# baaivision/Painter

Measured on AMD Instinct MI355X. Metric: images/sec (896x448 pairs) ViT-L fwd+bwd, higher is better.
Workload: dtype bf16; 1 GPU; painter_vit_large_patch16_input896x448 bf16 batch=8/GPU fwd+bwd on 1xMI355X (BASELINE configs[1]); global_batch=8, image=896x448x3 stitched pair, mode=train (DropPath 0.1), parallelism=dp1, rccl_ranks=0, backend=n/a, grad_allreduce=n/a

## Files before the change

include/painter_hip.h:

```cpp
#ifndef PAINTER_HIP_H
#define PAINTER_HIP_H

#include <stdint.h>

#ifdef __cplusplus
extern "C" {
#endif

#ifndef __HIP__
typedef struct ihipStream_t* hipStream_t;
#endif

enum { PA_F32 = 0, PA_BF16 = 1 };
enum {
    PA_EPI_BIAS = 0,
    PA_EPI_BIAS_F32 = 1,
    PA_EPI_BIAS_GELU = 2,
    PA_EPI_BIAS_RESID = 3
};

#define PA_ABI_VERSION 9
int pa_abi_version(void);
int pa_debug_set(int which, int value);
int pa_debug_get(int which);
// ... 5 lines not shown
int pa_linear_fwd_skip(int dtype, int epilogue, const void* x, int64_t ldx, const void* w, const float* bias, void* out, void* out2,
                       int64_t ldo, const float* resid, const float* rowscale, int rows_per_sample, int M, int N, int K,
                       const float* rowskip, int skip_rows_per_sample, hipStream_t stream);
int pa_linear_pixshuf(int dtype, const void* x, int64_t ldx, const void* w , const float* bias,
                      void* out_nhwc, int batch, int Hp, int Wp, int P, int C, int K, hipStream_t stream);
int64_t pa_linear_dgrad_workspace_bytes(int M, int K);
int pa_linear_dgrad(int dtype, const void* dy , int64_t lddy, const void* w ,
                    const void* gelu_aux , void* dx , int64_t lddx, float* dx_colsum,
                    void* workspace, int M, int N, int K, hipStream_t stream);
int pa_linear_dgrad_skip(int dtype, const void* dy, int64_t lddy, const void* w, const void* gelu_aux, void* dx, int64_t lddx, float* dx_colsum,
                         void* workspace, int M, int N, int K, const float* rowskip , int skip_rows_per_sample,
                         hipStream_t stream);
int64_t pa_linear_wgrad_workspace_bytes(int dtype, int M, int N, int K);
int pa_linear_wgrad(int dtype, const void* dy , int64_t lddy, const void* x , int64_t ldx,
                    float* dw , void* workspace, int M, int N, int K, hipStream_t stream);
int64_t pa_colsum_workspace_bytes(int M, int N);
int pa_colsum(int dtype, const void* x , int64_t ld, int M, int N, float* out , void* workspace,
              hipStream_t stream);
int pa_slab_reduce(const float* in, float* out, int64_t n, int nz, int64_t stride, int accumulate, hipStream_t stream);

int pa_layernorm_fwd(int dtype, const float* x, int64_t ldx, const float* gamma, const float* beta, float eps,
                     void* y , int64_t ldy, float* mean, float* rstd,
                     int R, int D, hipStream_t stream);
int64_t pa_layernorm_bwd_workspace_bytes(int R, int D);
int pa_layernorm_bwd(int dtype, const void* dy, int64_t lddy, const float* x, int64_t ldx, const float* mean,
                     const float* rstd, const float* gamma, const float* dres, float* dx, int64_t lddx, void* dxT,
                     int64_t lddxT, const float* rowscale, int rows_per_sample, float* dgamma_dbeta, float* dxT_colsum,
                     void* workspace, int R, int D, hipStream_t stream);
int pa_layernorm_bwd_reduce(const void* workspace, float* dgamma_dbeta, float* dxT_colsum, int with_colsum, int R, int D,
                            hipStream_t stream);
// ... 283 lines not shown
```

painter_amd/_lib.py:

```python
import ctypes
import os
import re

HERE = os.path.dirname(os.path.abspath(__file__))
HEADER = os.path.join(os.path.dirname(HERE), "include", "painter_hip.h")
LIB_PATH = os.environ.get("PAINTER_AMD_LIB") or os.path.join(HERE, "lib", "libpainter_hip.so")

PA_F32, PA_BF16 = 0, 1
EPI_BIAS, EPI_BIAS_F32, EPI_BIAS_GELU, EPI_BIAS_RESID = 0, 1, 2, 3
(KNOB_G256_STAGGER, KNOB_G256_NOSTORE, KNOB_G256_ORDER, KNOB_WGRAD_TARGET, KNOB_G256_SHORT_TILES, KNOB_G256_ILV, KNOB_RELPOS_SPLITS,
 KNOB_ATTN3_FUSE, KNOB_ATTN_LIGHT_LAST, KNOB_CONV_WGRAD_GROUPS, KNOB_LN_BWD_VARIANT, KNOB_G256_PATCH, KNOB_G256_MIXED) = range(13)
KNOB_G256_MIXED_NFULL, KNOB_DROP_SKIP, KNOB_DECODER_ROWS, KNOB_COUNT = 14, 16, 17, 18

_CT = {"int": ctypes.c_int, "int64_t": ctypes.c_int64, "float": ctypes.c_float, "double": ctypes.c_double, "hipStream_t": ctypes.c_void_p}


def parse_header(path=HEADER):
    src = open(path).read()
    src = re.sub(r"/\*.*?\*/", " ", src, flags=re.S)
    src = re.sub(r"//[^\n]*", " ", src)
    protos = {}
    for m in re.finditer(r"\b(int64_t|int)\s+(pa_\w+)\s*\(([^)]*)\)\s*;", src):
        ret, name, args = m.group(1), m.group(2), m.group(3).strip()
        argtypes = []
        if args and args != "void":
            for a in args.split(","):
                a = a.strip()
# ... 47 lines not shown
```

painter_amd/csrc/common.h:

```cpp
#pragma once
#include <hip/hip_runtime.h>
#include <stdint.h>
#include <cstdlib>

typedef __bf16 bf16;
typedef __attribute__((ext_vector_type(8))) __bf16 bf16x8;
typedef __attribute__((ext_vector_type(16))) float f32x16;

#define DEVI __device__ __forceinline__

template <typename T> struct TT;
template <> struct TT<float> {
    static constexpr int EPC = 4;
    static constexpr int BK = 32;
    static constexpr int KSTEPS = 2;
    static constexpr int SPF = 2;
    typedef uint4 Vec4;
};
template <> struct TT<bf16> {
    static constexpr int EPC = 8;
    static constexpr int BK = 64;
    static constexpr int KSTEPS = 4;
    static constexpr int SPF = 1;
    typedef uint2 Vec4;
// ... 69 lines not shown

enum Knob {
    KNOB_G256_STAGGER = 0,
    KNOB_G256_NOSTORE = 1,
    KNOB_G256_ORDER = 2,
    KNOB_WGRAD_TARGET = 3,
    KNOB_G256_SHORT_TILES = 4,
    KNOB_G256_ILV = 5,
    KNOB_RELPOS_SPLITS = 6,
    KNOB_ATTN3_FUSE = 7,
    KNOB_ATTN_LIGHT_LAST = 8,
    KNOB_CONV_WGRAD_GROUPS = 9,
    KNOB_LN_BWD_VARIANT = 10,
    KNOB_G256_PATCH = 11,
    KNOB_G256_MIXED = 12,
    KNOB_FREE_13 = 13,
    KNOB_G256_MIXED_NFULL = 14,
    KNOB_FREE_15 = 15,
    KNOB_DROP_SKIP = 16,
    KNOB_DECODER_ROWS = 17,
    KNOB_COUNT = 18
};
inline int g_knob[KNOB_COUNT] = {};
static inline bool drop_skip_on() {
    static const int env = [] { const char* v = getenv("PAINTER_AMD_DROP_SKIP"); return v ? atoi(v) : 1; }();
    return g_knob[KNOB_DROP_SKIP] == 1 ? false : (g_knob[KNOB_DROP_SKIP] == 2 ? true : env != 0);
}
static inline bool decoder_rows_on() {
    static const int env = [] { const char* v = getenv("PAINTER_AMD_DECODER_ROWS"); return v ? atoi(v) : 1; }();
    return g_knob[KNOB_DECODER_ROWS] == 1 ? false : (g_knob[KNOB_DECODER_ROWS] == 2 ? true : env != 0);
}

inline long long g_attn_counts[6] = {0, 0, 0, 0, 0, 0};
// ... 84 lines not shown
```

painter_amd/csrc/gemm.hip:

```cpp
#include <cstdlib>
#include "gemm_engine.h"
#include "gemm256.h"
#include "../../include/painter_hip.h"

template <typename OutT> struct EpiBias {
    OutT* out; size_t ldo; const float* bias; int M, N;
    DEVI void operator()(const f32x16 (&acc)[2][2], int ib, int jb, int lane, int) const {
        foreach_acc(acc, ib, jb, lane, [&](int i, int j, float v) {
            if (i < M && j < N) out[(size_t)i * ldo + j] = from_f<OutT>(v + (bias ? bias[j] : 0.f));
        });
    }
};
constexpr float G8_OFF = 0.13f, G8_SCALE = 255.f / 1.26f, G8_STEP = 1.26f / 255.f;
DEVI uint32_t g8_code(float g) { return min((uint32_t)fmaf(g, G8_SCALE, G8_OFF * G8_SCALE + 0.5f), 255u); }
DEVI float g8_value(uint32_t q) { return fmaf((float)q, G8_STEP, -G8_OFF); }
template <typename T> struct GeluAux { typedef T type; };
template <> struct GeluAux<bf16> { typedef unsigned char type; };
template <typename T> struct EpiBiasGelu {
    typename GeluAux<T>::type* aux; T* act; size_t ld; const float* bias; int M, N;
    DEVI void operator()(const f32x16 (&acc)[2][2], int ib, int jb, int lane, int) const {
        foreach_acc(acc, ib, jb, lane, [&](int i, int j, float v) {
            if (i < M && j < N) {
                const T p = from_f<T>(v + bias[j]);
                if constexpr (std::is_same<T, bf16>::value) {
// ... 490 lines not shown
extern "C" int pa_linear_dgrad(int dtype, const void* dy, int64_t lddy, const void* w, const void* gelu_aux,
                               void* dx, int64_t lddx, float* dx_colsum, void* workspace, int M, int N, int K, hipStream_t st) {
    return pa_linear_dgrad_skip(dtype, dy, lddy, w, gelu_aux, dx, lddx, dx_colsum, workspace, M, N, K, nullptr, 1, st);
}

static bool wgrad_fast(int dtype, int M, int N, int K) {
    return dtype == PA_BF16 && g256::ok(N, K, M, true, true, N, K) && K % 4 == 0 && N % 256 == 0 && K % 256 == 0;
}
static int wgrad_fast_splits(int M, int N, int K) {
    const int tiles = (N / 256) * (K / 256);
    static const int env_target = [] { const char* v = getenv("PA_WGRAD_WGS"); return v ? atoi(v) : 0; }();
    int target = env_target > 0 ? env_target : (g_knob[KNOB_WGRAD_TARGET] > 0 ? g_knob[KNOB_WGRAD_TARGET] : 256);
    if (target < 16) target = 16;
    int s = (target + 3 * tiles / 4) / tiles;
    if (s < 1) s = 1;
    const int ktiles = M / 64;
    if (s > ktiles / 4) s = ktiles / 4 > 0 ? ktiles / 4 : 1;
    return g256::splits_used(M, s);
}
static int wgrad_splits(int M, int N, int K, int bk) {
    const int tiles = ((N + 127) / 128) * ((K + 127) / 128);
    const int nku = (M + bk - 1) / bk;
    int s = (640 + tiles - 1) / tiles;
    if (s > nku) s = nku;
    if (s > 64) s = 64;
    if (s < 1) s = 1;
    return s;
}
extern "C" int64_t pa_linear_wgrad_workspace_bytes(int dtype, int M, int N, int K) {
    if (wgrad_fast(dtype, M, N, K)) {
        const int s = wgrad_fast_splits(M, N, K);
        return s > 1 ? (int64_t)s * N * K * sizeof(float) : 0;
    }
    const int s = wgrad_splits(M, N, K, dtype == PA_BF16 ? 64 : 32);
    return s > 1 ? (int64_t)s * N * K * sizeof(float) : 0;
}
template <typename T>
static int linear_wgrad_t(const T* dy, int64_t lddy, const T* x, int64_t ldx, float* dw, float* ws, int M, int N, int K,
                          hipStream_t st) {
    if constexpr (std::is_same<T, bf16>::value) {
        if (wgrad_fast(PA_BF16, M, N, K) && g256::ok(N, K, M, true, true, lddy, ldx)) {
            const int s = wgrad_fast_splits(M, N, K);
            if (s == 1) return g256::launch<true, true>(dy, lddy, x, ldx, Epi4Slab{dw, (size_t)K, 0, N, K}, N, K, M, 1, st);
            int e = g256::launch<true, true>(dy, lddy, x, ldx, Epi4Slab{ws, (size_t)K, (size_t)N * K, N, K}, N, K, M, s, st);
            if (e) return e;
            return pa_slab_reduce(ws, dw, (int64_t)N * K, s, (int64_t)N * K, 0, st);
        }
    }
    OpT<T> A{dy, (size_t)lddy, N, 0};
    OpT<T> B{x, (size_t)ldx, K, 0};
    const int s = wgrad_splits(M, N, K, TT<T>::BK);
    if (s == 1) return launch_gemm<T, 2, 2>(A, B, EpiSlab{dw, (size_t)K, 0, N, K}, N, K, M, 1, 1, st);
    int e = launch_gemm<T, 2, 2>(A, B, EpiSlab{ws, (size_t)K, (size_t)N * K, N, K}, N, K, M, s, 1, st);
    if (e) return e;
    return pa_slab_reduce(ws, dw, (int64_t)N * K, s, (int64_t)N * K, 0, st);
}
extern "C" int pa_linear_wgrad(int dtype, const void* dy, int64_t lddy, const void* x, int64_t ldx, float* dw,
                               void* workspace, int M, int N, int K, hipStream_t st) {
    if (N % 4 || K % 4) return (int)hipErrorInvalidValue;
    if (dtype == PA_BF16) return linear_wgrad_t<bf16>((const bf16*)dy, lddy, (const bf16*)x, ldx, dw, (float*)workspace, M, N, K, st);
    return linear_wgrad_t<float>((const float*)dy, lddy, (const float*)x, ldx, dw, (float*)workspace, M, N, K, st);
}

extern "C" int pa_fill_dead_rows(void* x, int64_t pitch_bytes, int64_t row_bytes, const int* rowmap, int M, hipStream_t st);
extern "C" int pa_linear_dgrad_live(const void* dy, int64_t lddy, const void* w, void* dx, int64_t lddx, const int* live, const int* rowmap,
                                    const int* count, int M, int N, int K, hipStream_t st) {
    if (live == nullptr || rowmap == nullptr || count == nullptr || M < 8 || K % 8 || lddx % 8) return (int)hipErrorInvalidValue;
    if (!g256::ok(M, K, N, false, true, lddy, K)) return (int)hipErrorInvalidValue;
    int e = pa_fill_dead_rows(dx, lddx * 2, (int64_t)K * 2, rowmap, M, st);
    if (e) return e;
    return g256::launch_live<false, true>((const bf16*)dy, lddy, (const bf16*)w, K, Epi4Scatter{(bf16*)dx, (size_t)lddx, live, count, M, K}, M, K, N, count, st);
}
extern "C" int pa_linear_wgrad_live(const void* dy, int64_t lddy, const void* x, int64_t ldx, float* dw, const int* count, int M, int N, int K,
                                    hipStream_t st) {
    if (count == nullptr || M < 128 || M % 128) return (int)hipErrorInvalidValue;
    if (!wgrad_fast(PA_BF16, M, N, K) || !g256::ok(N, K, M, true, true, lddy, ldx)) return (int)hipErrorInvalidValue;
// ... 13 lines not shown
```

painter_amd/csrc/gemm256.h:

```cpp
#pragma once
#include "common.h"
#include <cstdlib>
#include <type_traits>

namespace g256 {

constexpr int BM = 256, BN = 256, BK = 64, NT = 512;
constexpr int LDS_BYTES = 131072;
typedef __attribute__((address_space(3))) void lds_void;
typedef __attribute__((address_space(1))) const void gbl_cvoid;

DEVI constexpr int unit_off(bool isB, int sub, int stage) { return (isB ? 65536 : 0) + sub * 32768 + stage * 16384; }

template <int N> DEVI void wait_vm() { asm volatile("s_waitcnt vmcnt(%0)" ::"n"(N) : "memory"); }
DEVI void wait_lgkm0() { asm volatile("s_waitcnt lgkmcnt(0)" ::: "memory"); }

template <bool MM, bool IS_A>
DEVI uint32_t src_off(int tid, int j, int sub, int tile0, int rows, uint32_t ld) {
    const int cidx = j * NT + tid;
    if constexpr (!MM) {
        const int u = cidx >> 3, p = cidx & 7;
        const int kc = p ^ ((u >> 1) & 7);
        int row = IS_A ? ((u >> 6) * 128 + sub * 64 + (u & 63)) : ((u >> 5) * 64 + sub * 32 + (u & 31));
        row = min(tile0 + row, rows - 1);
// ... 51 lines not shown
    template <int KS> DEVI bf16x8 k() const {
        typedef __attribute__((ext_vector_type(2))) uint32_t u2;
        typedef __attribute__((ext_vector_type(4))) uint32_t u4;
        const uint2 l = KS == 0 ? l0 : KS == 1 ? l1 : KS == 2 ? l2 : l3;
        const uint2 h = KS == 0 ? h0 : KS == 1 ? h1 : KS == 2 ? h2 : h3;
        u2 lv = {l.x, l.y}, hv = {h.x, h.y};
        return __builtin_bit_cast(bf16x8, __builtin_shufflevector(lv, hv, 0, 1, 2, 3));
    }
};

template <class Epi> struct epi_colsum { static constexpr bool value = false; };
template <class Epi, class = void> struct epi_hi_off { static constexpr int value = 4; };
template <class Epi> struct epi_hi_off<Epi, std::void_t<decltype(Epi::HI_OFF)>> { static constexpr int value = Epi::HI_OFF; };
constexpr int BM_SHORT = 224;
constexpr int BM_HALF = 128;
template <bool AMM, bool BMM, int ILV, class Epi, bool SHORT = false, bool MIXED = false, bool SKIP = false, bool LIVE = false>
__global__ __launch_bounds__(NT) void gemm256_kernel(const bf16* __restrict__ Ag, uint32_t lda, const bf16* __restrict__ Bg,
                                                      uint32_t ldb, Epi epi, int M, int N, int ktiles, int ktiles_per_split,
                                                      int tiles_n, int stagger, int order, int nfull, int patch,
                                                      const float* __restrict__ rowskip, int rps, const int* __restrict__ live_count) {
    static_assert(!(LIVE && (SHORT || MIXED || SKIP)), "a device-side count goes with uniform 256-row tiles");
    static_assert(!(SHORT && AMM), "the 224-row tile is built for a K-major A operand");
    static_assert(!(SKIP && AMM), "row tiles are skipped only for a K-major A operand");
    static_assert(!(MIXED && (AMM || SHORT)), "half tiles are built for a K-major A operand and 256-row full tiles");
    constexpr int BMR = SHORT ? BM_SHORT : BM;
    extern __shared__ __attribute__((aligned(1024))) unsigned char smem[];
    const int tid = threadIdx.x, lane = tid & 63;
    if (stagger > 0 && blockIdx.x < 256 && blockIdx.y == 0) {
        const int64_t wait = ((int64_t)stagger * (((blockIdx.x >> 3) * 5) & 15)) >> 4;
        const uint64_t t0 = __builtin_amdgcn_s_memtime();
        while ((int64_t)(__builtin_amdgcn_s_memtime() - t0) < wait) __builtin_amdgcn_s_sleep(16);
    }
    const int wv = __builtin_amdgcn_readfirstlane(tid >> 6);
    const int wr = wv >> 2, wc = wv & 3;

    const bool htile = MIXED && (int)blockIdx.x >= nfull * tiles_n;
    int nwg = MIXED ? (htile ? (int)gridDim.x - nfull * tiles_n : nfull * tiles_n) : (int)gridDim.x;
    if constexpr (LIVE) {
        if constexpr (AMM) {
            ktiles = ktiles_per_split = min(ktiles, ((*live_count + 127) >> 7) * 2);
        } else {
            M = min(M, *live_count);
// ... 67 lines not shown
        if (skipped) {
            const int d = bid - nwg;
            int r = d / tiles_n;
            tn = d - r * tiles_n;
            bool found = false;
            skipped_ranges([&](int a, int b) {
                if (!found && r < b - a) { tm = a + r; found = true; }
                if (!found) r -= b - a;
            });
        } else {
            skipped_ranges([&](int a, int b) { if (tm >= a) tm += b - a; });
        }
    }
    const int i0 = htile ? nfull * BMR + tm * BM_HALF : tm * BMR, j0 = tn * BN;
    const bool blk3 = !(SHORT && wr == 1);
    const int kt0 = split * ktiles_per_split;
    const int nt = min(ktiles - kt0, ktiles_per_split);
    const bool empty = LIVE && AMM && nt == 0;
    uint32_t oa[2][2], ob[2][2];
#pragma unroll
    for (int sub = 0; sub < 2; ++sub)
#pragma unroll
        for (int j = 0; j < 2; ++j) {
            oa[sub][j] = src_off<AMM, true>(tid, j, sub, i0, M, lda);
            ob[sub][j] = src_off<BMM, false>(tid, j, sub, j0, N, ldb);
        }
    const size_t a_step = AMM ? (size_t)BK * lda * 2 : (size_t)BK * 2;
    const size_t b_step = BMM ? (size_t)BK * ldb * 2 : (size_t)BK * 2;
    const unsigned char* abase = reinterpret_cast<const unsigned char*>(Ag) + (size_t)kt0 * a_step;
    const unsigned char* bbase = reinterpret_cast<const unsigned char*>(Bg) + (size_t)kt0 * b_step;
    unsigned char* const dma_dst = smem + wv * 1024;

    auto piece_a = [&](int sub, int stage, int kt, int j) {
        const unsigned char* s = sgpr_ptr(abase + (size_t)kt * a_step);
        dma16(s + oa[sub][j], dma_dst + unit_off(false, sub, stage) + j * 8192);
    };
    auto piece_b = [&](int sub, int stage, int kt, int j) {
        const unsigned char* s = sgpr_ptr(bbase + (size_t)kt * b_step);
        dma16(s + ob[sub][j], dma_dst + unit_off(true, sub, stage) + j * 8192);
    };
    auto stage_a = [&](int sub, int stage, int kt) { piece_a(sub, stage, kt, 0); piece_a(sub, stage, kt, 1); };
    auto stage_b = [&](int sub, int stage, int kt) { piece_b(sub, stage, kt, 0); piece_b(sub, stage, kt, 1); };

    uint32_t ra[4], rb[4];
    {
// ... 48 lines not shown
    auto pre = [&](auto&& d0, auto&& d1) {
        if constexpr (ILV < 2) d0();
        if constexpr (ILV < 1) d1();
        wait_vm<8 - ILV>();
    };
    auto bar = [&]() {
        __builtin_amdgcn_sched_barrier(0);
        __builtin_amdgcn_s_barrier();
        __builtin_amdgcn_sched_barrier(0);
    };
    auto lwait = [&]() {
        wait_lgkm0();
        __builtin_amdgcn_sched_barrier(0);
    };

    auto tile_body = [&](auto stage_c, int T) {
        constexpr int S = decltype(stage_c)::value;
        const int t1 = min(T + 1, nt - 1), t2 = min(T + 2, nt - 1);
        fa0.template read<unit_off(false, 0, S)>(ra, 0);
        fa1.template read<unit_off(false, 0, S) + (AMM ? 0 : 4096)>(ra, 1);
        fb0.template read<unit_off(true, 0, S) - 65536>(rb, 0);
        {
            auto d0 = [&] { piece_b(1, S ^ 1, t1, 0); };
            auto d1 = [&] { piece_b(1, S ^ 1, t1, 1); };
            pre(d0, d1);
            bar(); lwait();
            mma_quad(0, 0, fb0, d0, d1);
            bar();
        }
        fb1.template read<unit_off(true, 1, S) - 65536>(rb, 0);
        {
            auto d0 = [&] { piece_a(1, S ^ 1, t1, 0); };
            auto d1 = [&] { piece_a(1, S ^ 1, t1, 1); };
// ... 60 lines not shown
    if constexpr (MIXED) {
        if (htile) {
            ran_half = true;
            if (!skipped) {
                piece_a(0, 0, 0, 0); piece_a(1, 0, 0, 0); stage_b(0, 0, 0); stage_b(1, 0, 0);
                wait_vm<0>();
                bar();
                for (int T = 0; T < nt; T += 2) {
                    half_body(I0{}, T);
                    half_body(I1{}, T + 1);
                }
            }
        }
    }
    if (!ran_half && !skipped && !empty) {
        stage_a(0, 0, 0);
        stage_b(0, 0, 0);
        stage_b(1, 0, 0);
        stage_a(1, 0, 0);
        stage_a(0, 1, 1);
        stage_b(0, 1, 1);
        wait_vm<8>();
        bar();
        if (wr == 1) bar();

        for (int T = 0; T < nt; T += 2) {
            tile_body(I0{}, T);
            tile_body(I1{}, T + 1);
        }
    }
    if (wr == 0 && !ran_half && !skipped && !empty) bar();
    wait_vm<0>();

    bar();
    {
        float* stg = reinterpret_cast<float*>(smem + wv * 8704);
// ... 45 lines not shown
                float v = cs[e];
                v += lane_dpp<0x128>(v);
                v += lane_xor16(v);
                v += lane_xor32(v);
                cs[e] = v;
            }
            if (lane < 8) epi.colsum_out((htile ? nfull + tm : tm) * 2 + wr, jcol, cs);
        }
    }
}

static inline int per_split(int ktiles, int nsplit) {
    int per = (ktiles + nsplit - 1) / nsplit;
    return per + (per & 1);
}
template <bool AMM, bool BMM, int ILV, bool SHORT, class Epi, bool MIXED = false, bool SKIP = false, bool LIVE = false>
static int launch_ilv(const bf16* A, size_t lda, const bf16* B, size_t ldb, Epi epi, int M, int N, int K, int nsplit, hipStream_t st, int nfull = 0,
                      const float* rowskip = nullptr, int rps = 1, const int* live_count = nullptr);
#ifndef G256_ILV_DEFAULT
#define G256_ILV_DEFAULT 2
#endif
static inline bool use_short(int M, int N, int nsplit, bool amm) {
    if (amm || nsplit != 1 || M < BM) return false;
    if (g_knob[KNOB_G256_SHORT_TILES] == 1) return false;
    if (g_knob[KNOB_G256_SHORT_TILES] == 2) return true;
    static const int cost = [] { const char* v = getenv("PA_G256_SHORT_COST"); return v ? atoi(v) : 92; }();
    const int tiles_n = (N + BN - 1) / BN;
    const long t256 = (long)((M + BM - 1) / BM) * tiles_n, t224 = (long)((M + BM_SHORT - 1) / BM_SHORT) * tiles_n;
    const long r256 = (t256 + 255) / 256 * 100, r224 = (t224 + 255) / 256 * cost;
    return r224 < r256;
}
// ... 35 lines not shown
    return launch_ilv<AMM, BMM, G256_ILV_DEFAULT, false>(A, lda, B, ldb, epi, M, N, K, nsplit, st);
#endif
}
template <bool BMM, class Epi>
static int launch_skip(const bf16* A, size_t lda, const bf16* B, size_t ldb, Epi epi, int M, int N, int K, hipStream_t st, const float* rowskip, int rps) {
    if ((M + rps - 1) / rps > 63) return launch<false, BMM>(A, lda, B, ldb, epi, M, N, K, 1, st);
    const TilePlan tp = tile_plan(M, N, 1, false);
    if (tp.mixed) return launch_ilv<false, BMM, G256_ILV_DEFAULT, false, Epi, true, true>(A, lda, B, ldb, epi, M, N, K, 1, st, tp.nfull, rowskip, rps);
    if (tp.is_short) return launch_ilv<false, BMM, G256_ILV_DEFAULT, true, Epi, false, true>(A, lda, B, ldb, epi, M, N, K, 1, st, 0, rowskip, rps);
    return launch_ilv<false, BMM, G256_ILV_DEFAULT, false, Epi, false, true>(A, lda, B, ldb, epi, M, N, K, 1, st, 0, rowskip, rps);
}
template <bool AMM, bool BMM, class Epi>
static int launch_live(const bf16* A, size_t lda, const bf16* B, size_t ldb, Epi epi, int M, int N, int K, const int* live_count, hipStream_t st) {
    return launch_ilv<AMM, BMM, G256_ILV_DEFAULT, false, Epi, false, false, true>(A, lda, B, ldb, epi, M, N, K, 1, st, 0, nullptr, 1, live_count);
}
template <bool AMM, bool BMM, int ILV, bool SHORT, class Epi, bool MIXED, bool SKIP, bool LIVE>
static int launch_ilv(const bf16* A, size_t lda, const bf16* B, size_t ldb, Epi epi, int M, int N, int K, int nsplit, hipStream_t st, int nfull,
                      const float* rowskip, int rps, const int* live_count) {
    auto kern = gemm256_kernel<AMM, BMM, ILV, Epi, SHORT, MIXED, SKIP, LIVE>;
    static bool attr_done = false;
    if (!attr_done) {
        hipError_t e = hipFuncSetAttribute(reinterpret_cast<const void*>(kern), hipFuncAttributeMaxDynamicSharedMemorySize, LDS_BYTES);
        if (e != hipSuccess) return (int)e;
        attr_done = true;
    }
    constexpr int BMR = SHORT ? BM_SHORT : BM;
    static const int env_patch = [] { const char* v = getenv("PA_G256_PATCH"); return v ? atoi(v) : 0; }();
    const int tiles_n = (N + BN - 1) / BN;
    const int tiles_m = MIXED ? nfull + (M - nfull * BMR + BM_HALF - 1) / BM_HALF : (M + BMR - 1) / BMR;
    const int ktiles = K / BK;
    const int per = per_split(ktiles, nsplit);
    const int splits = (ktiles + per - 1) / per;
    if (g_knob[KNOB_G256_NOSTORE]) epi.M = 0;
    PA_LAUNCH(kern, dim3(tiles_m * tiles_n, splits), dim3(NT), LDS_BYTES, st, A, (uint32_t)lda, B, (uint32_t)ldb, epi, M, N,
// ... 24 lines not shown
```

painter_amd/engine.py:

```python
import os
from typing import NamedTuple

import torch

from . import hostmath, ops
from ._lib import EPI_BIAS, EPI_BIAS_F32, EPI_BIAS_RESID, KNOB_RELPOS_SPLITS, KNOB_WGRAD_TARGET


_SIDE_STREAM = os.environ.get("PAINTER_AMD_SIDE_STREAM", "1") != "0"
_DBG_SERIAL = os.environ.get("PAINTER_AMD_DEBUG_SERIAL", "0") == "1"
_DBG_TRACE = os.environ.get("PAINTER_AMD_DEBUG_TRACE", "0") == "1"
_configured = False
WGRAD_SIDE_TARGET = 96
RELPOS_SIDE_SPLITS = 8


def _configure_library():
    global _configured
    if _configured:
        return
    from ._lib import lib
    lib.pa_debug_set(KNOB_RELPOS_SPLITS, RELPOS_SIDE_SPLITS if _SIDE_STREAM else 0)
    lib.pa_debug_set(KNOB_WGRAD_TARGET, WGRAD_SIDE_TARGET if _SIDE_STREAM else 0)
    _configured = True
# ... 113 lines not shown


class _Backward:
    __slots__ = ("P", "S", "sync", "want", "st", "G", "flats", "rc_shape", "dnorm")

    def __init__(self, P, S, sync, want, st):
        self.P, self.S, self.sync, self.want, self.st = P, S, sync, want, st
        self.G = {}
        self.flats = {}
        self.rc_shape = tuple(S.blocks[-1].rcat.shape)
        self.dnorm = None

    def need(self, n):
        return self.want is None or n in self.want

    def param_grads(self, wname, bname, dy, x, bout=None, wgrad=None, colsum=None):
        G = self.G
        do_w, do_b = self.need(wname), bname not in G and self.need(bname)
        if not (do_w or do_b):
            return

        def fn():
            if do_w:
                G[wname] = (wgrad or ops.linear_wgrad)(dy, x)
            if do_b:
                G[bname] = (colsum or ops.colsum)(dy, out=bout)
        self.st.run(fn, dy, x if do_w else None)

    def ready(self, names, flat=None):
        self.st.ready(self.sync, self.G, names, flat=flat)


class HotPath:

    def __init__(self, cfg: HotPathConfig, compute_dtype):
        self.cfg = cfg
        self.T = compute_dtype
        self._M = None
        self._wcache = {}
# ... 285 lines not shown
        flat, fl = self.block_flat(X, i)
        del X.flats[i]
        if i in c.taps:
            k = c.taps.index(i)
            tap = S.taps[k]
            dyT = torch.empty((R, D), dtype=T, device=dev)
            dx, gb = ops.layernorm_bwd(dconcat[:, k * D:(k + 1) * D], tap.x, tap.mean, tap.rstd, P["norm.weight"], dres=dx, dx=dx, dxT=dyT,
                                       rowscale=ds_m, rows_per_sample=L, dxT_colsum=fl["fc2"])
            G[pre + "mlp.fc2.bias"] = fl["fc2"]
            if need("norm.weight") or need("norm.bias"):
                X.dnorm = gb if X.dnorm is None else _add_(X.dnorm, gb)
        elif i == c.merge_idx:
            dx, dyT = ops.merge_bwd(T, dx, ds_m, L, B * L, D)
        else:
            dyT = dyT_next
        X.param_grads(pre + "mlp.fc2.weight", pre + "mlp.fc2.bias", dyT, b.act, fl["fc2"])
        tr("%d.dyT" % i, dyT)
        dpre = ops.linear_dgrad(dyT, self.w(pre + "mlp.fc2.weight", P), gelu_aux=b.gaux, colsum_out=fl["fc1"], rowskip=ds_m, rows_per_sample=L)
        G[pre + "mlp.fc1.bias"] = fl["fc1"]
        tr("%d.dpre" % i, dpre)
        X.param_grads(pre + "mlp.fc1.weight", pre + "mlp.fc1.bias", dpre, b.ln2, fl["fc1"])
        dln2 = ops.linear_dgrad(dpre, self.w(pre + "mlp.fc1.weight", P), rowskip=ds_m, rows_per_sample=L)
        tr("%d.dln2" % i, dln2)
        del dpre
        dyA = st.private(dyT)
        lnws, lndone = self.ln_workspace(dev, ops.layernorm_bwd_workspace_bytes(R, D), st.main, st.side)
        dx, fin = ops.layernorm_bwd(dln2, b.x1, b.mean2, b.rstd2, P[pre + "norm2.weight"], dres=dx, dx=dx, dxT=dyA,
                                    rowscale=ds_a, rows_per_sample=L, gb=fl["n2"].view(2, D), dxT_colsum=fl["proj"], defer=True, ws=lnws)
        gb = None
        if need(pre + "norm2.weight") or need(pre + "norm2.bias") or need(pre + "attn.proj.bias"):
            gb = st.run(fin)
            lndone()
            G[pre + "norm2.weight"], G[pre + "norm2.bias"] = gb[0], gb[1]
        G[pre + "attn.proj.bias"] = fl["proj"]
        del dyT
        tr("%d.dx_ln2" % i, dx); tr("%d.dyA" % i, dyA)
        if gb is not None:
            tr("%d.gb2" % i, gb)
        if b.group > 0:
            da = ops.ensemble_resid(torch.zeros_like(dx), dx if ds_a is None else ops.scale_cast(torch.float32, dx, ds_a, L), b.Bc, b.group, L, D)
            dyA = da if T == torch.float32 else ops.cast_bf16(da, out=dyA)
            del da
        X.param_grads(pre + "attn.proj.weight", pre + "attn.proj.bias", dyA, b.ao, fl["proj"])
        dao = ops.linear_dgrad(dyA, self.w(pre + "attn.proj.weight", P), out=dln2, rowskip=sk_a, rows_per_sample=L)
        tr("%d.dao" % i, dao)
        del dyA
        rcatT = self.relpos(pre, P, True)
        dqkv, dG = ops.attn_bwd_core(b.qkv, b.rcat, rcatT, b.ao, dao, b.lse, b.Bc, L, c.heads, c.Hp, c.Wp, c.scale, tables=b.atab, rowskip=sk_a)
        if need(pre + "attn.rel_pos_h") or need(pre + "attn.rel_pos_w"):
            drcat = st.run(lambda: ops.attn_bwd_relpos(dG, b.qkv, nrp, b.Bc, L, c.heads, c.Hp, c.Wp, out=fl["rel"].view(nrp, hd)), dG, b.qkv)
            nh, nw = 2 * c.Hp - 1, 2 * c.Wp - 1
            G[pre + "attn.rel_pos_h"] = drcat[:nh]
            G[pre + "attn.rel_pos_w"] = drcat[nh:nh + nw]
        del dG
        tr("%d.dqkv" % i, dqkv)
        X.param_grads(pre + "attn.qkv.weight", pre + "attn.qkv.bias", dqkv, b.ln1, fl["qkv"])
        dln1 = ops.linear_dgrad(dqkv, self.w(pre + "attn.qkv.weight", P), out=dao, rowskip=sk_a, rows_per_sample=L)
        del dqkv
        nxt = i - 1
        if nxt >= 0 and nxt not in c.taps and nxt != c.merge_idx:
            dyT_next = torch.empty((R, D), dtype=T, device=dev)
        else:
            dyT_next = None
        ds_next = None if (S.drop is None or nxt < 0) else S.drop[nxt][1]
        cs_next = None
        if dyT_next is not None:
            cs_next = self.block_flat(X, nxt)[1]["fc2"]
            G["blocks.%d.mlp.fc2.bias" % nxt] = cs_next
        lnws, lndone = self.ln_workspace(dev, ops.layernorm_bwd_workspace_bytes(R, D), st.main, st.side)
        dx, fin = ops.layernorm_bwd(dln1, b.x, b.mean1, b.rstd1, P[pre + "norm1.weight"], dres=dx, dx=dx, dxT=dyT_next,
                                    rowscale=ds_next if dyT_next is not None else None, rows_per_sample=L, gb=fl["n1"].view(2, D),
# ... 52 lines not shown
```

painter_amd/ops.py:

```python
import torch

from ._lib import (EPI_BIAS, EPI_BIAS_F32, EPI_BIAS_GELU, EPI_BIAS_RESID, KNOB_DECODER_ROWS, KNOB_DROP_SKIP, PA_BF16, PA_F32, check, lib)

_WS = {}


def stream():
    return torch.cuda.current_stream().cuda_stream


def code(dtype):
    if dtype == torch.bfloat16:
        return PA_BF16
    if dtype == torch.float32:
        return PA_F32
    raise TypeError("painter_amd supports float32 / bfloat16 operand types, got %s" % dtype)


def p(t):
    return 0 if t is None else t.data_ptr()


def workspace(nbytes, device, slot=0):
    key = (device, slot, torch.cuda.current_stream(device).cuda_stream)
# ... 103 lines not shown
    _req(dy); _req(w, T)
    if out is None:
        out = torch.empty((M, K), dtype=T, device=dy.device)
    if gelu_aux is not None:
        assert gelu_aux.stride(0) == out.stride(0) and gelu_aux.dtype == gelu_aux_dtype(T), (gelu_aux.dtype, gelu_aux.stride(0), out.stride(0))
    ws = None
    if colsum_out is not None:
        assert colsum_out.shape == (K,) and colsum_out.dtype == torch.float32 and colsum_out.is_contiguous()
        ws = workspace(lib.pa_linear_dgrad_workspace_bytes(M, K), dy.device, slot=2)
    sk, srps = _skip_args(rowskip, rows_per_sample, M)
    check(lib.pa_linear_dgrad_skip(code(T), p(dy), dy.stride(0), p(w), p(gelu_aux), p(out), out.stride(0), p(colsum_out), p(ws), M, N, K,
                                   sk, srps, stream()), "pa_linear_dgrad_skip")
    return out


def linear_wgrad(dy, x, out=None, *, live=None):
    if live is not None:
        lv, count = live
        return linear_wgrad_live(dy, gather_rows(x, lv, count), count, out=out)
    M, N = dy.shape
    K = x.shape[1]
    T = dy.dtype
    _req(dy); _req(x, T)
    if out is None:
        out = torch.empty((N, K), dtype=torch.float32, device=dy.device)
    ws = workspace(lib.pa_linear_wgrad_workspace_bytes(code(T), M, N, K), dy.device)
    check(lib.pa_linear_wgrad(code(T), p(dy), dy.stride(0), p(x), x.stride(0), p(out), p(ws), M, N, K, stream()),
          "pa_linear_wgrad")
    return out


def colsum(x, out=None):
    M, N = x.shape
    if out is None:
        out = torch.empty((N,), dtype=torch.float32, device=x.device)
    ws = workspace(lib.pa_colsum_workspace_bytes(M, N), x.device)
    check(lib.pa_colsum(code(x.dtype), p(x), x.stride(0), M, N, p(out), p(ws), stream()), "pa_colsum")
    return out


def decoder_rows(mode=None):
    return _knob(KNOB_DECODER_ROWS, mode)


# ... 399 lines not shown
```

Before: 166.6 images/sec.

## Skip dropped-sample contraction tiles in weight-gradient GEMMs under DropPath

```diff
diff --git a/include/painter_hip.h b/include/painter_hip.h
--- a/include/painter_hip.h
+++ b/include/painter_hip.h
@@ -43,6 +43,9 @@
 int64_t pa_linear_wgrad_workspace_bytes(int dtype, int M, int N, int K);
 int pa_linear_wgrad(int dtype, const void* dy , int64_t lddy, const void* x , int64_t ldx,
                     float* dw , void* workspace, int M, int N, int K, hipStream_t stream);
+int pa_linear_wgrad_skip(int dtype, const void* dy, int64_t lddy, const void* x, int64_t ldx, float* dw, void* workspace, int M, int N, int K,
+                         const float* rowskip, int rows_per_sample, hipStream_t stream);
+int pa_wgrad_skip_tiles(const float* factors, int M, int rows_per_sample, int nsplit, int balanced, int* counts, int* tiles);
 int64_t pa_colsum_workspace_bytes(int M, int N);
 int pa_colsum(int dtype, const void* x , int64_t ld, int M, int N, float* out , void* workspace,
               hipStream_t stream);
diff --git a/painter_amd/_lib.py b/painter_amd/_lib.py
--- a/painter_amd/_lib.py
+++ b/painter_amd/_lib.py
@@ -10,7 +10,7 @@
 EPI_BIAS, EPI_BIAS_F32, EPI_BIAS_GELU, EPI_BIAS_RESID = 0, 1, 2, 3
 (KNOB_G256_STAGGER, KNOB_G256_NOSTORE, KNOB_G256_ORDER, KNOB_WGRAD_TARGET, KNOB_G256_SHORT_TILES, KNOB_G256_ILV, KNOB_RELPOS_SPLITS,
  KNOB_ATTN3_FUSE, KNOB_ATTN_LIGHT_LAST, KNOB_CONV_WGRAD_GROUPS, KNOB_LN_BWD_VARIANT, KNOB_G256_PATCH, KNOB_G256_MIXED) = range(13)
-KNOB_G256_MIXED_NFULL, KNOB_DROP_SKIP, KNOB_DECODER_ROWS, KNOB_COUNT = 14, 16, 17, 18
+KNOB_WGRAD_SKIP_BALANCED, KNOB_G256_MIXED_NFULL, KNOB_WGRAD_SPLITS, KNOB_DROP_SKIP, KNOB_DECODER_ROWS, KNOB_COUNT = 13, 14, 15, 16, 17, 18
 
 _CT = {"int": ctypes.c_int, "int64_t": ctypes.c_int64, "float": ctypes.c_float, "double": ctypes.c_double, "hipStream_t": ctypes.c_void_p}
 
diff --git a/painter_amd/csrc/common.h b/painter_amd/csrc/common.h
--- a/painter_amd/csrc/common.h
+++ b/painter_amd/csrc/common.h
@@ -107,9 +107,9 @@
     KNOB_LN_BWD_VARIANT = 10,
     KNOB_G256_PATCH = 11,
     KNOB_G256_MIXED = 12,
-    KNOB_FREE_13 = 13,
+    KNOB_WGRAD_SKIP_BALANCED = 13,
     KNOB_G256_MIXED_NFULL = 14,
-    KNOB_FREE_15 = 15,
+    KNOB_WGRAD_SPLITS = 15,
     KNOB_DROP_SKIP = 16,
     KNOB_DECODER_ROWS = 17,
     KNOB_COUNT = 18
diff --git a/painter_amd/csrc/gemm.hip b/painter_amd/csrc/gemm.hip
--- a/painter_amd/csrc/gemm.hip
+++ b/painter_amd/csrc/gemm.hip
@@ -528,6 +528,7 @@
     if (target < 16) target = 16;
     int s = (target + 3 * tiles / 4) / tiles;
     if (s < 1) s = 1;
+    if (g_knob[KNOB_WGRAD_SPLITS] > 0) s = g_knob[KNOB_WGRAD_SPLITS];
     const int ktiles = M / 64;
     if (s > ktiles / 4) s = ktiles / 4 > 0 ? ktiles / 4 : 1;
     return g256::splits_used(M, s);
@@ -551,10 +552,16 @@
 }
 template <typename T>
 static int linear_wgrad_t(const T* dy, int64_t lddy, const T* x, int64_t ldx, float* dw, float* ws, int M, int N, int K,
-                          hipStream_t st) {
+                          hipStream_t st, const float* rowskip = nullptr, int skip_rps = 1) {
     if constexpr (std::is_same<T, bf16>::value) {
         if (wgrad_fast(PA_BF16, M, N, K) && g256::ok(N, K, M, true, true, lddy, ldx)) {
             const int s = wgrad_fast_splits(M, N, K);
+            if (rowskip != nullptr) {
+                if (s == 1) return g256::launch_wskip(dy, lddy, x, ldx, Epi4Slab{dw, (size_t)K, 0, N, K}, N, K, M, 1, st, rowskip, skip_rps);
+                int e = g256::launch_wskip(dy, lddy, x, ldx, Epi4Slab{ws, (size_t)K, (size_t)N * K, N, K}, N, K, M, s, st, rowskip, skip_rps);
+                if (e) return e;
+                return pa_slab_reduce(ws, dw, (int64_t)N * K, s, (int64_t)N * K, 0, st);
+            }
             if (s == 1) return g256::launch<true, true>(dy, lddy, x, ldx, Epi4Slab{dw, (size_t)K, 0, N, K}, N, K, M, 1, st);
             int e = g256::launch<true, true>(dy, lddy, x, ldx, Epi4Slab{ws, (size_t)K, (size_t)N * K, N, K}, N, K, M, s, st);
             if (e) return e;
@@ -574,6 +581,29 @@
     if (N % 4 || K % 4) return (int)hipErrorInvalidValue;
     if (dtype == PA_BF16) return linear_wgrad_t<bf16>((const bf16*)dy, lddy, (const bf16*)x, ldx, dw, (float*)workspace, M, N, K, st);
     return linear_wgrad_t<float>((const float*)dy, lddy, (const float*)x, ldx, dw, (float*)workspace, M, N, K, st);
+}
+extern "C" int pa_linear_wgrad_skip(int dtype, const void* dy, int64_t lddy, const void* x, int64_t ldx, float* dw, void* workspace, int M, int N,
+                                    int K, const float* rowskip, int rows_per_sample, hipStream_t st) {
+    if (N % 4 || K % 4) return (int)hipErrorInvalidValue;
+    if (rowskip != nullptr && rows_per_sample < 1) return (int)hipErrorInvalidValue;
+    if (!drop_skip_on()) rowskip = nullptr;
+    if (dtype == PA_BF16) return linear_wgrad_t<bf16>((const bf16*)dy, lddy, (const bf16*)x, ldx, dw, (float*)workspace, M, N, K, st, rowskip, rows_per_sample);
+    return linear_wgrad_t<float>((const float*)dy, lddy, (const float*)x, ldx, dw, (float*)workspace, M, N, K, st);
+}
+extern "C" int pa_wgrad_skip_tiles(const float* factors, int M, int rows_per_sample, int nsplit, int balanced, int* counts, int* tiles) {
+    if (factors == nullptr || counts == nullptr || tiles == nullptr || rows_per_sample < 1 || nsplit < 1 || M < 128 || M % 128) return -1;
+    const int ktiles = M / g256::BK, per = g256::per_split(ktiles, nsplit), splits = g256::splits_used(M, nsplit);
+    const int ns = (int)(((long long)M + rows_per_sample - 1) / rows_per_sample);
+    unsigned long long dmask = 0;
+    if (ns <= 63)
+        for (int s = 0; s < ns; ++s) dmask |= (unsigned long long)(factors[s] == 0.f) << s;
+    for (int s = 0; s < splits; ++s) {
+        int p0, nt;
+        const g256::KeptTiles k = g256::split_tiles(dmask, rows_per_sample, ktiles, per, s, splits, balanced != 0, p0, nt);
+        counts[s] = nt;
+        for (int t = 0; t < nt; ++t) tiles[(size_t)s * ktiles + t] = g256::kept_tile(k, p0 + t, ktiles);
+    }
+    return splits;
 }
 
 extern "C" int pa_fill_dead_rows(void* x, int64_t pitch_bytes, int64_t row_bytes, const int* rowmap, int M, hipStream_t st);
diff --git a/painter_amd/csrc/gemm256.h b/painter_amd/csrc/gemm256.h
--- a/painter_amd/csrc/gemm256.h
+++ b/painter_amd/csrc/gemm256.h
@@ -89,18 +89,101 @@
 template <class Epi> struct epi_hi_off<Epi, std::void_t<decltype(Epi::HI_OFF)>> { static constexpr int value = Epi::HI_OFF; };
 constexpr int BM_SHORT = 224;
 constexpr int BM_HALF = 128;
-template <bool AMM, bool BMM, int ILV, class Epi, bool SHORT = false, bool MIXED = false, bool SKIP = false, bool LIVE = false>
+constexpr int WS_RUNS = 4, WS_HEAD = 2;
+struct KeptTiles {
+    int thr[WS_RUNS];
+    int len[WS_RUNS];
+    int lo;
+    int kept, dead;
+};
+__host__ __device__ inline KeptTiles kept_tiles(unsigned long long dmask, int rps, int lo, int hi, int head) {
+    KeptTiles k;
+    const int lo_h = lo + head;
+    const unsigned sfirst = (unsigned)lo_h * BK / (unsigned)rps;
+    unsigned long long m = dmask & (~0ull << (sfirst < 63 ? sfirst : 63));
+    int dead = 0;
+#pragma unroll
+    for (int r = 0; r < WS_RUNS; ++r) {
+        int a = lo_h, b = lo_h;
+        if (m != 0) {
+            const int s0 = __builtin_ctzll(m), s1 = s0 + __builtin_ctzll(~(m >> s0));
+            m &= ~0ull << s1;
+            const long long ta = ((long long)s0 * rps + BK - 1) / BK, tb = (long long)s1 * rps / BK;
+            a = (int)(ta < lo_h ? lo_h : ta > hi ? hi : ta);
+            b = (int)(tb < lo_h ? lo_h : tb > hi ? hi : tb);
+            if (b < a) b = a;
+        }
+        k.thr[r] = a - lo - dead;
+        k.len[r] = b - a;
+        dead += b - a;
+    }
+    const int odd = (hi - lo - dead) & 1;
+    int adj = 0;
+#pragma unroll
+    for (int r = 0; r < WS_RUNS; ++r) {
+        k.thr[r] += adj;
+        const int take = (odd != 0 && adj == 0 && k.len[r] > 0) ? 1 : 0;
+        k.len[r] -= take;
+        adj |= take;
+    }
+    k.lo = lo;
+    k.dead = dead - adj;
+    k.kept = hi - lo - k.dead;
+    return k;
+}
+__host__ __device__ inline int kept_tile(const KeptTiles& k, int p, int ktiles) {
+    int t = k.lo + p;
+#pragma unroll
+    for (int r = 0; r < WS_RUNS; ++r) t += p >= k.thr[r] ? k.len[r] : 0;
+    t = t < ktiles - 1 ? t : ktiles - 1;
+    return t > 0 ? t : 0;
+}
+__host__ __device__ inline KeptTiles split_tiles(unsigned long long dmask, int rps, int ktiles, int per, int split, int nsplits, bool balanced,
+                                                 int& p0, int& nt) {
+    const int lo = split * per < ktiles ? split * per : ktiles, hi = lo + per < ktiles ? lo + per : ktiles;
+    if (dmask == 0) {
+        KeptTiles k;
+#pragma unroll
+        for (int r = 0; r < WS_RUNS; ++r) k.thr[r] = k.len[r] = 0;
+        k.lo = lo;
+        k.kept = hi - lo;
+        k.dead = 0;
+        p0 = 0;
+        nt = hi - lo;
+        return k;
+    }
+    if (balanced) {
+        const KeptTiles k = kept_tiles(dmask, rps, 0, ktiles, 0);
+        if (k.dead != 0) {
+            const int pairs = k.kept >> 1, q = pairs / nsplits, r = pairs - q * nsplits;
+            p0 = 2 * (split * q + (split < r ? split : r));
+            nt = 2 * (q + (split < r ? 1 : 0));
+            return k;
+        }
+    }
+    const KeptTiles k = kept_tiles(dmask, rps, lo, hi, WS_HEAD);
+    p0 = 0;
+    nt = k.kept;
+    return k;
+}
+template <bool AMM, bool BMM, int ILV, class Epi, bool SHORT = false, bool MIXED = false, bool SKIP = false, bool LIVE = false, bool WSKIP = false>
 __global__ __launch_bounds__(NT) void gemm256_kernel(const bf16* __restrict__ Ag, uint32_t lda, const bf16* __restrict__ Bg,
                                                       uint32_t ldb, Epi epi, int M, int N, int ktiles, int ktiles_per_split,
                                                       int tiles_n, int stagger, int order, int nfull, int patch,
                                                       const float* __restrict__ rowskip, int rps, const int* __restrict__ live_count) {
     static_assert(!(LIVE && (SHORT || MIXED || SKIP)), "a device-side count goes with uniform 256-row tiles");
+    static_assert(!WSKIP || (AMM && !SHORT && !MIXED && !SKIP && !LIVE), "contraction tiles are left out only for an M-major A operand, on plain tiles");
     static_assert(!(SHORT && AMM), "the 224-row tile is built for a K-major A operand");
     static_assert(!(SKIP && AMM), "row tiles are skipped only for a K-major A operand");
     static_assert(!(MIXED && (AMM || SHORT)), "half tiles are built for a K-major A operand and 256-row full tiles");
     constexpr int BMR = SHORT ? BM_SHORT : BM;
     extern __shared__ __attribute__((aligned(1024))) unsigned char smem[];
     const int tid = threadIdx.x, lane = tid & 63;
+    [[maybe_unused]] float wskip_f = 1.f;
+    if constexpr (WSKIP) {
+        const int ns = (int)(((long long)ktiles * BK + rps - 1) / rps);
+        if (lane < ns) wskip_f = rowskip[lane];
+    }
     if (stagger > 0 && blockIdx.x < 256 && blockIdx.y == 0) {
         const int64_t wait = ((int64_t)stagger * (((blockIdx.x >> 3) * 5) & 15)) >> 4;
         const uint64_t t0 = __builtin_amdgcn_s_memtime();
@@ -198,9 +281,23 @@
     }
     const int i0 = htile ? nfull * BMR + tm * BM_HALF : tm * BMR, j0 = tn * BN;
     const bool blk3 = !(SHORT && wr == 1);
-    const int kt0 = split * ktiles_per_split;
-    const int nt = min(ktiles - kt0, ktiles_per_split);
-    const bool empty = LIVE && AMM && nt == 0;
+    int kt0_ = split * ktiles_per_split;
+    int nt_ = min(ktiles - kt0_, ktiles_per_split);
+    [[maybe_unused]] KeptTiles kmap;
+    const bool wbal = WSKIP && nfull != 0;
+    auto wskip_map = [&]() {
+        asm volatile("" : "+v"(wskip_f)::"memory");
+        kmap = split_tiles(__ballot(wskip_f == 0.f), rps, ktiles, ktiles_per_split, split, (int)gridDim.y, wbal, kt0_, nt_);
+    };
+    if constexpr (WSKIP) {
+        if (wbal) wskip_map();
+    }
+    const int &kt0 = kt0_, &nt = nt_;
+    const bool empty = ((LIVE && AMM) || WSKIP) && nt == 0;
+    auto ktile = [&](int t) {
+        if constexpr (WSKIP) return kept_tile(kmap, kt0 + t, ktiles);
+        else return t;
+    };
     uint32_t oa[2][2], ob[2][2];
 #pragma unroll
     for (int sub = 0; sub < 2; ++sub)
@@ -211,8 +308,8 @@
         }
     const size_t a_step = AMM ? (size_t)BK * lda * 2 : (size_t)BK * 2;
     const size_t b_step = BMM ? (size_t)BK * ldb * 2 : (size_t)BK * 2;
-    const unsigned char* abase = reinterpret_cast<const unsigned char*>(Ag) + (size_t)kt0 * a_step;
-    const unsigned char* bbase = reinterpret_cast<const unsigned char*>(Bg) + (size_t)kt0 * b_step;
+    const unsigned char* abase = reinterpret_cast<const unsigned char*>(Ag) + (WSKIP ? 0 : (size_t)kt0 * a_step);
+    const unsigned char* bbase = reinterpret_cast<const unsigned char*>(Bg) + (WSKIP ? 0 : (size_t)kt0 * b_step);
     unsigned char* const dma_dst = smem + wv * 1024;
 
     auto piece_a = [&](int sub, int stage, int kt, int j) {
@@ -291,9 +388,17 @@
         __builtin_amdgcn_sched_barrier(0);
     };
 
+    [[maybe_unused]] int wnext = 0;
     auto tile_body = [&](auto stage_c, int T) {
         constexpr int S = decltype(stage_c)::value;
-        const int t1 = min(T + 1, nt - 1), t2 = min(T + 2, nt - 1);
+        int t1, t2;
+        if constexpr (WSKIP) {
+            t1 = wnext;
+            t2 = wnext = ktile(min(T + 2, nt - 1));
+        } else {
+            t1 = min(T + 1, nt - 1);
+            t2 = min(T + 2, nt - 1);
+        }
         fa0.template read<unit_off(false, 0, S)>(ra, 0);
         fa1.template read<unit_off(false, 0, S) + (AMM ? 0 : 4096)>(ra, 1);
         fb0.template read<unit_off(true, 0, S) - 65536>(rb, 0);
@@ -384,12 +489,17 @@
         }
     }
     if (!ran_half && !skipped && !empty) {
-        stage_a(0, 0, 0);
-        stage_b(0, 0, 0);
-        stage_b(1, 0, 0);
-        stage_a(1, 0, 0);
-        stage_a(0, 1, 1);
-        stage_b(0, 1, 1);
+        const int k0 = (WSKIP && !wbal) ? kt0 : ktile(0), k1 = (WSKIP && !wbal) ? kt0 + 1 : ktile(1);
+        stage_a(0, 0, k0);
+        stage_b(0, 0, k0);
+        stage_b(1, 0, k0);
+        stage_a(1, 0, k0);
+        stage_a(0, 1, k1);
+        stage_b(0, 1, k1);
+        if constexpr (WSKIP) {
+            if (!wbal) wskip_map();
+            wnext = ktile(1);
+        }
         wait_vm<8>();
         bar();
         if (wr == 1) bar();
@@ -465,7 +575,7 @@
     int per = (ktiles + nsplit - 1) / nsplit;
     return per + (per & 1);
 }
-template <bool AMM, bool BMM, int ILV, bool SHORT, class Epi, bool MIXED = false, bool SKIP = false, bool LIVE = false>
+template <bool AMM, bool BMM, int ILV, bool SHORT, class Epi, bool MIXED = false, bool SKIP = false, bool LIVE = false, bool WSKIP = false>
 static int launch_ilv(const bf16* A, size_t lda, const bf16* B, size_t ldb, Epi epi, int M, int N, int K, int nsplit, hipStream_t st, int nfull = 0,
                       const float* rowskip = nullptr, int rps = 1, const int* live_count = nullptr);
 #ifndef G256_ILV_DEFAULT
@@ -531,10 +641,16 @@
 static int launch_live(const bf16* A, size_t lda, const bf16* B, size_t ldb, Epi epi, int M, int N, int K, const int* live_count, hipStream_t st) {
     return launch_ilv<AMM, BMM, G256_ILV_DEFAULT, false, Epi, false, false, true>(A, lda, B, ldb, epi, M, N, K, 1, st, 0, nullptr, 1, live_count);
 }
-template <bool AMM, bool BMM, int ILV, bool SHORT, class Epi, bool MIXED, bool SKIP, bool LIVE>
+template <class Epi>
+static int launch_wskip(const bf16* A, size_t lda, const bf16* B, size_t ldb, Epi epi, int M, int N, int K, int nsplit, hipStream_t st, const float* rowskip, int rps) {
+    if (((long long)K + rps - 1) / rps > 63) return launch<true, true>(A, lda, B, ldb, epi, M, N, K, nsplit, st);
+    const int balanced = g_knob[KNOB_WGRAD_SKIP_BALANCED] == 1;
+    return launch_ilv<true, true, G256_ILV_DEFAULT, false, Epi, false, false, false, true>(A, lda, B, ldb, epi, M, N, K, nsplit, st, balanced, rowskip, rps);
+}
+template <bool AMM, bool BMM, int ILV, bool SHORT, class Epi, bool MIXED, bool SKIP, bool LIVE, bool WSKIP>
 static int launch_ilv(const bf16* A, size_t lda, const bf16* B, size_t ldb, Epi epi, int M, int N, int K, int nsplit, hipStream_t st, int nfull,
                       const float* rowskip, int rps, const int* live_count) {
-    auto kern = gemm256_kernel<AMM, BMM, ILV, Epi, SHORT, MIXED, SKIP, LIVE>;
+    auto kern = gemm256_kernel<AMM, BMM, ILV, Epi, SHORT, MIXED, SKIP, LIVE, WSKIP>;
     static bool attr_done = false;
     if (!attr_done) {
         hipError_t e = hipFuncSetAttribute(reinterpret_cast<const void*>(kern), hipFuncAttributeMaxDynamicSharedMemorySize, LDS_BYTES);
diff --git a/painter_amd/engine.py b/painter_amd/engine.py
--- a/painter_amd/engine.py
+++ b/painter_amd/engine.py
@@ -151,7 +151,7 @@
     def need(self, n):
         return self.want is None or n in self.want
 
-    def param_grads(self, wname, bname, dy, x, bout=None, wgrad=None, colsum=None):
+    def param_grads(self, wname, bname, dy, x, bout=None, wgrad=None, colsum=None, rowskip=None, rows_per_sample=1):
         G = self.G
         do_w, do_b = self.need(wname), bname not in G and self.need(bname)
         if not (do_w or do_b):
@@ -159,7 +159,7 @@
 
         def fn():
             if do_w:
-                G[wname] = (wgrad or ops.linear_wgrad)(dy, x)
+                G[wname] = wgrad(dy, x) if wgrad else ops.linear_wgrad(dy, x, rowskip=rowskip, rows_per_sample=rows_per_sample)
             if do_b:
                 G[bname] = (colsum or ops.colsum)(dy, out=bout)
         self.st.run(fn, dy, x if do_w else None)
@@ -475,12 +475,12 @@
             dx, dyT = ops.merge_bwd(T, dx, ds_m, L, B * L, D)
         else:
             dyT = dyT_next
-        X.param_grads(pre + "mlp.fc2.weight", pre + "mlp.fc2.bias", dyT, b.act, fl["fc2"])
+        X.param_grads(pre + "mlp.fc2.weight", pre + "mlp.fc2.bias", dyT, b.act, fl["fc2"], rowskip=ds_m, rows_per_sample=L)
         tr("%d.dyT" % i, dyT)
         dpre = ops.linear_dgrad(dyT, self.w(pre + "mlp.fc2.weight", P), gelu_aux=b.gaux, colsum_out=fl["fc1"], rowskip=ds_m, rows_per_sample=L)
         G[pre + "mlp.fc1.bias"] = fl["fc1"]
         tr("%d.dpre" % i, dpre)
-        X.param_grads(pre + "mlp.fc1.weight", pre + "mlp.fc1.bias", dpre, b.ln2, fl["fc1"])
+        X.param_grads(pre + "mlp.fc1.weight", pre + "mlp.fc1.bias", dpre, b.ln2, fl["fc1"], rowskip=ds_m, rows_per_sample=L)
         dln2 = ops.linear_dgrad(dpre, self.w(pre + "mlp.fc1.weight", P), rowskip=ds_m, rows_per_sample=L)
         tr("%d.dln2" % i, dln2)
         del dpre
@@ -502,7 +502,7 @@
             da = ops.ensemble_resid(torch.zeros_like(dx), dx if ds_a is None else ops.scale_cast(torch.float32, dx, ds_a, L), b.Bc, b.group, L, D)
             dyA = da if T == torch.float32 else ops.cast_bf16(da, out=dyA)
             del da
-        X.param_grads(pre + "attn.proj.weight", pre + "attn.proj.bias", dyA, b.ao, fl["proj"])
+        X.param_grads(pre + "attn.proj.weight", pre + "attn.proj.bias", dyA, b.ao, fl["proj"], rowskip=sk_a, rows_per_sample=L)
         dao = ops.linear_dgrad(dyA, self.w(pre + "attn.proj.weight", P), out=dln2, rowskip=sk_a, rows_per_sample=L)
         tr("%d.dao" % i, dao)
         del dyA
@@ -515,7 +515,7 @@
             G[pre + "attn.rel_pos_w"] = drcat[nh:nh + nw]
         del dG
         tr("%d.dqkv" % i, dqkv)
-        X.param_grads(pre + "attn.qkv.weight", pre + "attn.qkv.bias", dqkv, b.ln1, fl["qkv"])
+        X.param_grads(pre + "attn.qkv.weight", pre + "attn.qkv.bias", dqkv, b.ln1, fl["qkv"], rowskip=sk_a, rows_per_sample=L)
         dln1 = ops.linear_dgrad(dqkv, self.w(pre + "attn.qkv.weight", P), out=dao, rowskip=sk_a, rows_per_sample=L)
         del dqkv
         nxt = i - 1
diff --git a/painter_amd/ops.py b/painter_amd/ops.py
--- a/painter_amd/ops.py
+++ b/painter_amd/ops.py
@@ -141,8 +141,9 @@
     return out
 
 
-def linear_wgrad(dy, x, out=None, *, live=None):
+def linear_wgrad(dy, x, out=None, *, live=None, rowskip=None, rows_per_sample=1):
     if live is not None:
+        assert rowskip is None
         lv, count = live
         return linear_wgrad_live(dy, gather_rows(x, lv, count), count, out=out)
     M, N = dy.shape
@@ -152,9 +153,23 @@
     if out is None:
         out = torch.empty((N, K), dtype=torch.float32, device=dy.device)
     ws = workspace(lib.pa_linear_wgrad_workspace_bytes(code(T), M, N, K), dy.device)
-    check(lib.pa_linear_wgrad(code(T), p(dy), dy.stride(0), p(x), x.stride(0), p(out), p(ws), M, N, K, stream()),
-          "pa_linear_wgrad")
-    return out
+    sk, srps = _skip_args(rowskip, rows_per_sample, M)
+    check(lib.pa_linear_wgrad_skip(code(T), p(dy), dy.stride(0), p(x), x.stride(0), p(out), p(ws), M, N, K, sk, srps, stream()),
+          "pa_linear_wgrad_skip")
+    return out
+
+
+def wgrad_skip_tiles(factors, M, rows_per_sample, nsplit, balanced=False):
+    import ctypes
+    f = (ctypes.c_float * len(factors))(*[float(v) for v in factors])
+    if rows_per_sample < 1 or len(factors) * rows_per_sample < M or M < 128:
+        raise ValueError("wgrad_skip_tiles: bad arguments")
+    kt = M // 64
+    counts, tiles = (ctypes.c_int * kt)(), (ctypes.c_int * (kt * kt))()
+    n = lib.pa_wgrad_skip_tiles(ctypes.addressof(f), M, rows_per_sample, nsplit, int(bool(balanced)), ctypes.addressof(counts), ctypes.addressof(tiles))
+    if n < 0:
+        raise ValueError("pa_wgrad_skip_tiles: bad arguments")
+    return [[tiles[s * kt + t] for t in range(counts[s])] for s in range(n)]
 
 
 def colsum(x, out=None):
```

Result: no change. 166.4 images/sec (-0.1%).
